# vasabi-root/gaus-slam

Hardware: AMD Instinct MI355X
Metric: fwd+bwd frames/sec @ 640x480, 500k Gaussians (higher is better)
Workload: dtype f32

## Files before the change

gaus_slam_amd/csrc/gs2d_api.hip:

```cpp
#include "gs2d_common.h"
#include "../../include/gs2d_rasterizer.h"

#include <stdio.h>
#include <stdlib.h>
#include <string.h>
#include <chrono>
#include <string>
#include <atomic>
#include <mutex>
#include <thread>
#if defined(__x86_64__) || defined(__i386__)
#include <immintrin.h>
#endif

namespace {

thread_local std::string g_err;

int fail(const char* what, hipError_t e)
{
    char buf[512];
    snprintf(buf, sizeof(buf), "gs2d: %s: %s", what, hipGetErrorString(e));
    g_err = buf;
    return -1;
// ... 6 lines not shown

#define GS2D_CHECK(expr, what)                        \
    do {                                              \
        hipError_t _e = (expr);                       \
        if (_e != hipSuccess) return fail(what, _e);  \
    } while (0)

#define GS2D_STAGE(what)                                                             \
    do {                                                                             \
        hipError_t _e = hipGetLastError();                                           \
        if (_e != hipSuccess) return fail(what, _e);                                 \
        if (debug) { _e = hipStreamSynchronize(s); if (_e != hipSuccess) return fail(what, _e); } \
    } while (0)

uint32_t higher_msb(uint32_t n)
{
    uint32_t msb = sizeof(n) * 4, step = msb;
    while (step > 1) {
        step /= 2;
        if (n >> msb) msb += step; else msb -= step;
    }
    if (n >> msb) msb++;
    return msb;
}

enum { ST_PREPROCESS = 0, ST_SCAN, ST_DUPLICATE, ST_SORT, ST_RANGES, ST_BLEND_FWD, ST_BLEND_BWD, ST_PREPROCESS_BWD, ST_CULL, ST_COUNT };
struct StageTimer {
    bool enabled = false;
    hipEvent_t ev[ST_COUNT][2];
    bool have_ev = false;
    bool recorded[ST_COUNT] = {};
    void begin(int st, hipStream_t s)
    {
        if (!enabled) return;
        if (!have_ev) {
            for (int i = 0; i < ST_COUNT; i++) { (void)hipEventCreate(&ev[i][0]); (void)hipEventCreate(&ev[i][1]); }
            have_ev = true;
        }
        (void)hipEventRecord(ev[st][0], s);
    }
    void end(int st, hipStream_t s)
    {
        if (!enabled) return;
        (void)hipEventRecord(ev[st][1], s);
        recorded[st] = true;
    }
};
StageTimer g_timer;

std::atomic<int> g_deterministic{0};
std::atomic<int> g_reference_binning{0};
static int launch_ahead_default() { const char* e = getenv("GS2D_LAUNCH_AHEAD"); return (e && e[0] == '0') ? 0 : 1; }
std::atomic<int> g_launch_ahead{launch_ahead_default()};

struct PinnedWord {
    uint32_t* p = nullptr;
    ~PinnedWord() { if (p) (void)hipHostFree(p); }
};
thread_local PinnedWord g_pinned;
struct FwdRecord {
    const void* geom = nullptr;
    const void* bin = nullptr;
    size_t bin_bytes = 0;
    int det = 0, R = 0, P = 0;
    bool clean = false;
};
struct FwdTable {
    static constexpr int N = 64;
    std::mutex m;
    FwdRecord e[N];
    int next = 0;
    void drop(const void* geom) { std::lock_guard<std::mutex> l(m); for (auto& r : e) if (r.geom == geom) r = FwdRecord(); }
    void add(const FwdRecord& r) { std::lock_guard<std::mutex> l(m); e[next] = r; next = (next + 1) % N; }
    bool find(const void* geom, bool take_clean, FwdRecord* out)
    {
        std::lock_guard<std::mutex> l(m);
        for (auto& r : e)
            if (r.geom == geom && geom != nullptr) {
                *out = r;
                if (take_clean) r.clean = false;
                return true;
            }
        return false;
    }
};
FwdTable g_fwd;

struct LastCount { int P = -1, W = 0, H = 0; uint32_t R = 0; };
thread_local LastCount g_last[GS2D_MAX_BATCH];

inline void cpu_relax()
{
#if defined(__x86_64__) || defined(__i386__)
    _mm_pause();
#elif defined(__aarch64__)
    asm volatile("yield" ::: "memory");
#else
    std::this_thread::yield();
#endif
}

}

extern "C" {

const char* gs2d_last_error(void) { return g_err.c_str(); }

void gs2d_stage_timing_enable(int on)
{
    g_timer.enabled = on != 0;
    for (int i = 0; i < ST_COUNT; i++) g_timer.recorded[i] = false;
}

int gs2d_stage_timing_read(float ms[9])
{
    for (int i = 0; i < ST_COUNT; i++) {
        ms[i] = -1.f;
        if (!g_timer.recorded[i]) continue;
        if (hipEventSynchronize(g_timer.ev[i][1]) != hipSuccess) return -1;
        float t = 0.f;
        if (hipEventElapsedTime(&t, g_timer.ev[i][0], g_timer.ev[i][1]) != hipSuccess) return -1;
        ms[i] = t;
    }
    return 0;
}

int gs2d_stage_timing_read_abs(float ms[18])
{
    for (int i = 0; i < 2 * ST_COUNT; i++) ms[i] = -1.f;
    if (!g_timer.recorded[ST_PREPROCESS]) return 0;
    for (int i = 0; i < ST_COUNT; i++) {
        if (!g_timer.recorded[i]) continue;
        if (hipEventSynchronize(g_timer.ev[i][1]) != hipSuccess) return -1;
        for (int e = 0; e < 2; e++) {
            float t = 0.f;
            if (hipEventElapsedTime(&t, g_timer.ev[ST_PREPROCESS][0], g_timer.ev[i][e]) != hipSuccess) {
                if (hipEventElapsedTime(&t, g_timer.ev[i][e], g_timer.ev[ST_PREPROCESS][0]) != hipSuccess) return -1;
                t = -t;
            }
            ms[2 * i + e] = t;
        }
    }
    return 0;
}

void gs2d_set_deterministic(int on) { g_deterministic.store(on != 0); }
int gs2d_get_deterministic(void) { return g_deterministic.load(); }
void gs2d_set_reference_binning(int on) { g_reference_binning.store(on != 0); }
void gs2d_set_launch_ahead(int on) { g_launch_ahead.store(on != 0); }
int gs2d_get_launch_ahead(void) { return g_launch_ahead.load(); }
int gs2d_get_reference_binning(void) { return g_reference_binning.load(); }

#ifndef GS2D_SOURCE_HASH
#define GS2D_SOURCE_HASH "unknown"
#endif
const char* gs2d_build_info(void) { return "gs2d-hip gfx950 strict-fp (fp-contract=off) " __DATE__ " src " GS2D_SOURCE_HASH; }

size_t gs2d_geometry_bytes(int P) { return geom_layout(P).total; }
size_t gs2d_image_bytes(int width, int height) { return img_layout(width, height).total; }
size_t gs2d_binning_bytes(int R) { return bin_layout(R, g_deterministic.load() != 0).total; }

void gs2d_geometry_layout(int P, size_t o[5])
{
    const GeomLayout L = geom_layout(P);
    o[0] = L.depths; o[1] = L.tiles_touched; o[2] = L.point_offsets; o[3] = L.rec; o[4] = L.clamped;
}
void gs2d_binning_layout(int R, size_t o[2])
{
    const BinLayout L = bin_layout(R);
    o[0] = L.point_list; o[1] = L.keys;
}
size_t gs2d_binning_contrib_offset(int R) { return bin_layout(R, g_deterministic.load() != 0).contrib; }
void gs2d_image_layout(int width, int height, size_t o[2])
{
    const ImgLayout L = img_layout(width, height);
    o[0] = L.ranges; o[1] = L.pix;
}

}

namespace {

struct FwdShared {
    int P, D, M, width, height, use_sa, debug;
    const float* background;
    const float *means3D, *shs, *colors_precomp, *opacities, *scales, *rotations, *transMat_precomp;
    float scale_modifier;
    hipStream_t s;
};
struct FwdFrame {
    gs2d_alloc_fn geometry_alloc, binning_alloc, image_alloc;
    void *geometry_user, *binning_user, *image_user;
    const float *viewmatrix, *projmatrix, *cam_pos, *pose_Rt, *pose_quat;
    float* out_color; float* out_others; int* radii;
    char* geom = nullptr; char* bin = nullptr; char* img = nullptr;
    size_t bin_bytes = 0;
    GeomLayout GL; CamParams cam;
    volatile uint32_t* pinned = nullptr;
    bool fused_sort = false;
    int sort_cap = 0;
    bool spec = false;
    bool store_pending = false;
    bool ahead = false;
// ... 91 lines not shown
                                f.pose_Rt, f.pose_quat, scan_tmp, s);
    g_timer.end(ST_PREPROCESS, s);
    GS2D_STAGE("preprocess");

    if (!g_pinned.p) GS2D_CHECK(hipHostMalloc((void**)&g_pinned.p, 64, hipHostMallocCoherent), "hipHostMalloc");
    f.pinned = g_pinned.p + slot;
    f.spec = img_layout(c.width, c.height).tiles <= GS2D_BIN_MAX_TILES;
    if (f.spec) return 0;
    const int nblk = (c.P + 255) / 256;
    uint32_t* total_dev = scan_tmp + nblk + 8;
    *f.pinned = 0xFFFFFFFFu;
    g_timer.begin(ST_SCAN, s);
    gs2d::launch_offsets_blocksums(c.P, scan_tmp, total_dev, g_pinned.p + slot, s);
    g_timer.end(ST_SCAN, s);
    {
        const hipError_t le = hipGetLastError();
        if (le != hipSuccess) return fail("scan", le);
    }
    f.store_pending = true;
    return 0;
}

int fwd_phase_b(const FwdShared& c, FwdFrame& f, int slot, bool allow_ahead = true)
{
    const int debug = c.debug;
    hipStream_t s = c.s;
    const int P = c.P, width = c.width, height = c.height;
    const GeomLayout& GL = f.GL;
    const CamParams& cam = f.cam;
    const ImgLayout IL = img_layout(width, height);
    f.img = (char*)f.image_alloc(f.image_user, IL.total);
    if (!f.img) { (void)wait_total(f, s); return fail_msg("image allocation failed"); }
    LastCount& last = g_last[slot];
    const bool same_shape = last.P == P && last.W == width && last.H == height;
    const size_t guess_R = same_shape ? (size_t)last.R + last.R / 8 + 4096 : (size_t)P * 3 + 4096;
    const int C0 = (int)(guess_R > 0x7fffffffull ? 0x7fffffffull : guess_R);
    const bool det = g_deterministic.load() != 0;
    char* geom = f.geom;
    char* img = f.img;
    float* depths = (float*)(geom + GL.depths);
    uint32_t* tiles_touched = (uint32_t*)(geom + GL.tiles_touched);
    uint32_t* point_offsets = (uint32_t*)(geom + GL.point_offsets);
    ushort4* rect = (ushort4*)(geom + GL.rect);
    uint32_t* scan_tmp = (uint32_t*)(geom + GL.scan_tmp);
    int C = C0;
    const size_t pre_bytes = bin_layout(C0, det, C0).total;
    char* bin_pre = (char*)f.binning_alloc(f.binning_user, pre_bytes);
    if (f.spec) {
        if (!bin_pre) return fail_msg("binning allocation failed");
        const BinLayout B0 = bin_layout(C0, det, C0);
        *f.pinned = 0xFFFFFFFFu;
        const bool ahead = allow_ahead && g_launch_ahead.load() != 0 && !debug && !det;
        uint32_t* total_dev = scan_tmp + (P + 255) / 256 + 8;
        g_timer.begin(ST_DUPLICATE, s);
        gs2d::launch_duplicate(P, rect, depths, tiles_touched, scan_tmp, 0, point_offsets, cam.gx, (uint64_t*)(bin_pre + B0.keys_alt),
                               (uint32_t*)(bin_pre + B0.vals_alt), (uint32_t)C0, (uint32_t*)f.pinned, s, ahead ? total_dev : nullptr);
        g_timer.end(ST_DUPLICATE, s);
        {
            const hipError_t le = hipGetLastError();
            if (le != hipSuccess) return fail("duplicate", le);
        }
        f.store_pending = true;
        if (ahead) {
            const gs2d::DevBin db = {bin_pre, total_dev, (uint32_t)C0, 0};
            uint2* ranges = (uint2*)(img + IL.ranges);
            const int tile_bits = (int)higher_msb((uint32_t)(cam.gx * cam.gy));
            g_timer.begin(ST_SORT, s);
            gs2d::launch_bin_by_tile_dev(db, IL.tiles, tile_bits, ranges, s);
            const long long Rg = same_shape ? (long long)last.R : (long long)C0;
            const int cap_class = gs2d::tile_sort_capacity(Rg, IL.tiles);
            f.sort_cap = gs2d::gs2d_fused_sort_cap(cap_class);
            f.fused_sort = f.sort_cap > 0;
            if (!f.fused_sort) gs2d::launch_tile_depth_sort_dev(db, IL.tiles, ranges, cap_class, 0, s);
            g_timer.end(ST_SORT, s);
            GS2D_STAGE("bin by tile (count on the device)");
            f.ahead = true; f.cap = C0; f.det = false;
            f.bin = bin_pre;
            f.bf.ranges = ranges; f.bf.point_list = nullptr; f.bf.rec = (const float4*)(geom + GL.rec);
            f.bf.out_color = f.out_color; f.bf.out_others = f.out_others; f.bf.pix_state = (float*)(img + IL.pix);
            f.bf.hits = nullptr; f.bf.hits4 = nullptr; f.bf.contrib = nullptr; f.bf.zero = (float4*)(geom + GL.grad_rec);
            f.bf.keys = nullptr; f.bf.keys_alt = nullptr; f.bf.vals_alt = nullptr;
            f.bf.dev = db;
            return 0;
        }
    }
    if (!wait_total(f, s)) return fail_msg("num_rendered read-back failed");
    if (debug) GS2D_CHECK(hipStreamSynchronize(s), f.spec ? "duplicate" : "scan");
    const uint32_t num_rendered_u = *f.pinned;
    if (num_rendered_u == 0xFFFFFFFFu) return fail_msg("num_rendered read-back failed");
    if (num_rendered_u > 0x7fffffffu) return fail_msg("num_rendered overflows int32");
    const int R = (int)num_rendered_u;
    f.R = R;

    last.P = P; last.W = width; last.H = height; last.R = num_rendered_u;
    const bool reuse_pre = bin_pre && R <= C0;
    if (!reuse_pre) C = R;
    const BinLayout BL = bin_layout(R, det, C);
    char* bin = reuse_pre ? bin_pre : (char*)f.binning_alloc(f.binning_user, BL.total);
    if (!bin) return fail_msg("binning allocation failed");
    f.bin = bin;
    f.bin_bytes = BL.total;
    uint32_t* point_list = (uint32_t*)(bin + BL.point_list);
    uint64_t* keys = (uint64_t*)(bin + BL.keys);
    uint32_t* vals_alt = (uint32_t*)(bin + BL.vals_alt);
    uint64_t* keys_alt = (uint64_t*)(bin + BL.keys_alt);
    uint32_t* hist = (uint32_t*)(bin + BL.hist);
    uint2* ranges = (uint2*)(img + IL.ranges);

    const int tile_bits = (int)higher_msb((uint32_t)(cam.gx * cam.gy));
    const int end_bit = 32 + tile_bits;
    const bool one_pass = IL.tiles <= GS2D_BIN_MAX_TILES;
    const int passes = one_pass ? 1 : (end_bit - 32 + 7) / 8;
    uint64_t* k_unsorted = (passes & 1) ? keys_alt : keys;
    uint32_t* v_unsorted = (passes & 1) ? vals_alt : point_list;
    if (!f.spec) {
        g_timer.begin(ST_DUPLICATE, s);
        gs2d::launch_duplicate(P, rect, depths, tiles_touched, scan_tmp, 1, point_offsets, cam.gx, k_unsorted, v_unsorted, 0xFFFFFFFFu,
                               nullptr, s);
        g_timer.end(ST_DUPLICATE, s);
    } else if (!reuse_pre) {
        gs2d::launch_duplicate(P, rect, depths, tiles_touched, scan_tmp, 0, point_offsets, cam.gx, k_unsorted, v_unsorted, (uint32_t)C,
// ... 556 lines not shown
```

gaus_slam_amd/csrc/gs2d_binning.hip:

```cpp
#include "gs2d_common.h"
#include "gs2d_scan.h"
#include "gs2d_tile_sort.h"

#include <stdlib.h>

namespace {

__global__ void __launch_bounds__(SCAN_T) scan_reduce_kernel(const uint32_t* __restrict__ in, int n, uint32_t* __restrict__ block_sums)
{
    const int base = blockIdx.x * GS2D_SCAN_ITEMS + threadIdx.x * SCAN_PER_T;
    uint32_t s = 0;
#pragma unroll
    for (int i = 0; i < SCAN_PER_T; i++)
        if (base + i < n) s += in[base + i];
    uint32_t total;
    block_incl_scan(s, &total);
    if (threadIdx.x == 0) block_sums[blockIdx.x] = total;
}

__global__ void __launch_bounds__(SCAN_T) scan_blocksums_kernel(uint32_t* __restrict__ block_sums, int nblocks, uint32_t* __restrict__ total_out,
                                                                uint32_t* __restrict__ total_host)
{
    scan_blocksums_body(block_sums, nblocks, total_out, total_host);
}
// ... 359 lines not shown
bin_scatter_kernel(const uint64_t* __restrict__ keys_in, const uint32_t* __restrict__ vals_in, uint64_t* __restrict__ keys_out,
                   uint32_t* __restrict__ vals_out, int n, int ntiles, int nbits, const uint32_t* __restrict__ offs_excl,
                   const uint32_t* __restrict__ tile_total, int nblocks, uint2* __restrict__ ranges)
{
    bin_scatter_body<ITEMS>(keys_in, vals_in, keys_out, vals_out, n, ntiles, nbits, offs_excl, tile_total, nblocks, ranges);
}
__global__ void __launch_bounds__(BIN_T) bin_scatter_batch_kernel(int ntiles, int nbits, const gs2d::BinFrames tab)
{
    const gs2d::BinFrame& f = tab.f[blockIdx.y];
    if (f.nblocks == 0) return;
    bin_scatter_body<BIN_ITEMS>(f.keys_unsorted, f.vals_unsorted, f.keys, f.point_list, f.R, ntiles, nbits, f.hist,
                                f.hist + (size_t)ntiles * f.nblocks, f.nblocks, f.ranges);
}

struct DevBinPtrs {
    int R, nblocks;
    const uint64_t* keys_unsorted; const uint32_t* vals_unsorted;
    uint64_t* keys; uint32_t* point_list; uint64_t* keys_alt; uint32_t* vals_alt; uint32_t* hist;
};
__device__ __forceinline__ bool dev_bin_ptrs(const gs2d::DevBin& db, DevBinPtrs* o, int items)
{
    const uint32_t R = *db.R_dev;
    if (R > db.cap) return false;
    const BinLayout L = bin_layout((int)R, db.det != 0, (int)db.cap);
    o->R = (int)R;
    o->nblocks = ((int)R + items - 1) / items;
    o->keys = (uint64_t*)(db.base + L.keys); o->point_list = (uint32_t*)(db.base + L.point_list);
    o->keys_alt = (uint64_t*)(db.base + L.keys_alt); o->vals_alt = (uint32_t*)(db.base + L.vals_alt);
    o->keys_unsorted = o->keys_alt; o->vals_unsorted = o->vals_alt;
    o->hist = (uint32_t*)(db.base + L.hist);
    return true;
}
template <int ITEMS>
__global__ void __launch_bounds__(BIN_T) bin_hist_dev_kernel(const gs2d::DevBin db, int ntiles)
{
    DevBinPtrs p;
    if (!dev_bin_ptrs(db, &p, ITEMS)) return;
    bin_hist_body<ITEMS>(p.keys_unsorted, p.R, ntiles, p.hist, p.nblocks);
}
__global__ void __launch_bounds__(256) bin_row_scan_dev_kernel(const gs2d::DevBin db, int ntiles, int items)
{
    DevBinPtrs p;
    if (!dev_bin_ptrs(db, &p, items)) return;
    bin_row_scan_body(p.hist, ntiles, p.nblocks, p.hist + (size_t)ntiles * p.nblocks);
}
template <int ITEMS>
__global__ void __launch_bounds__(BIN_T) bin_scatter_dev_kernel(const gs2d::DevBin db, int ntiles, int nbits, uint2* __restrict__ ranges)
{
    DevBinPtrs p;
    if (!dev_bin_ptrs(db, &p, ITEMS)) return;
    bin_scatter_body<ITEMS>(p.keys_unsorted, p.vals_unsorted, p.keys, p.point_list, p.R, ntiles, nbits, p.hist,
                     p.hist + (size_t)ntiles * p.nblocks, p.nblocks, ranges);
}
__global__ void __launch_bounds__(256)
tile_depth_sort_dev_kernel(const gs2d::DevBin db, const uint2* __restrict__ ranges, int cap, int write_keys)
{
    extern __shared__ uint32_t dyn[];
    __shared__ uint32_t wcnt[4][256];
    DevBinPtrs p;
    if (!dev_bin_ptrs(db, &p, BIN_ITEMS) || p.R == 0) return;
    tile_depth_sort_body(blockIdx.x, dyn, wcnt, ranges, p.keys, p.point_list, p.keys_alt, p.vals_alt, cap, 1, write_keys);
}

__global__ void __launch_bounds__(256)
tile_depth_sort_kernel(const uint2* __restrict__ ranges, uint64_t* __restrict__ keys, uint32_t* __restrict__ vals,
                       uint64_t* __restrict__ keys_alt, uint32_t* __restrict__ vals_alt, int cap, int packed, int write_keys)
{
    extern __shared__ uint32_t dyn[];
    __shared__ uint32_t wcnt[4][256];
    tile_depth_sort_body(blockIdx.x, dyn, wcnt, ranges, keys, vals, keys_alt, vals_alt, cap, packed, write_keys);
}
__global__ void __launch_bounds__(256) tile_depth_sort_batch_kernel(int cap, int write_keys, const gs2d::BinFrames tab)
{
    const gs2d::BinFrame& f = tab.f[blockIdx.y];
    extern __shared__ uint32_t dyn[];
    __shared__ uint32_t wcnt[4][256];
    if (f.R > 0) tile_depth_sort_body(blockIdx.x, dyn, wcnt, f.ranges, f.keys, f.point_list, f.keys_alt, f.vals_alt, cap, 1, write_keys);
}

__global__ void __launch_bounds__(256) tile_ranges_kernel(int L, const uint64_t* __restrict__ keys, uint2* __restrict__ ranges)
{
    const int idx = blockIdx.x * 256 + threadIdx.x;
    if (idx >= L) return;
    const uint32_t cur = (uint32_t)(keys[idx] >> 32);
    if (idx == 0) ranges[cur].x = 0;
    else {
        const uint32_t prev = (uint32_t)(keys[idx - 1] >> 32);
        if (cur != prev) { ranges[prev].y = idx; ranges[cur].x = idx; }
    }
    if (idx == L - 1) ranges[cur].y = L;
}

}

namespace gs2d {

int bin_items_for(long long count, int tiles)
{
    static const int forced = [] { const char* e = getenv("GS2D_BIN_ITEMS_FORCE"); return e ? atoi(e) : 0; }();
    if (forced == 4096 || forced == 8192 || forced == 16384) return forced;
    return tiles > 2560 && count >= 8192LL * 128 ? 8192 : BIN_ITEMS;
}

static size_t bin_lds_bytes(int tiles) { return 4 * (size_t)(tiles + 2 * (tiles + (tiles & 1))); }
static int bin_grid(int nblocks) { return nblocks > 0 ? 8 * ((nblocks + 7) / 8) : 1; }

// ... 24 lines not shown
                      uint32_t capacity, uint32_t* total_host, hipStream_t s, uint32_t* total_dev)
{
    hipLaunchKernelGGL(duplicate_kernel, dim3((P + 255) / 256), dim3(256), 0, s, P, rect, depths, tiles_touched, block_sums, scanned,
                       point_offsets, gx, keys, vals, capacity, total_host, total_dev);
}

void launch_sort_pairs(int R, uint64_t* keys_a, uint32_t* vals_a, uint64_t* keys_b, uint32_t* vals_b, int begin_bit,
                       int end_bit, uint32_t* hist, size_t hist_elems, hipStream_t s)
{
    if (R <= 0) return;
    const int nblocks = (R + GS2D_SORT_ITEMS - 1) / GS2D_SORT_ITEMS;
    uint32_t* scan_tmp = hist + hist_elems;
    const int passes = (end_bit - begin_bit + 7) / 8;
    uint64_t* kin = (passes & 1) ? keys_b : keys_a;
    uint32_t* vin = (passes & 1) ? vals_b : vals_a;
    uint64_t* kout = (passes & 1) ? keys_a : keys_b;
    uint32_t* vout = (passes & 1) ? vals_a : vals_b;
    for (int p = 0; p < passes; p++) {
        const int shift = begin_bit + 8 * p;
        hipLaunchKernelGGL(radix_hist_kernel, dim3(nblocks), dim3(SORT_T), 0, s, kin, R, shift, hist, nblocks);
        launch_inclusive_scan(hist, hist, (int)hist_elems, scan_tmp, nullptr, s);
        hipLaunchKernelGGL(radix_scatter_kernel, dim3(nblocks), dim3(SORT_T), 0, s, kin, vin, kout, vout, R, shift, hist,
                           nblocks);
        uint64_t* tk = kin; kin = kout; kout = tk;
        uint32_t* tv = vin; vin = vout; vout = tv;
    }
}

bool launch_bin_by_tile(int R, int tiles, int nbits, const uint64_t* keys_in, const uint32_t* vals_in, uint64_t* keys_out,
                        uint32_t* vals_out, uint32_t* hist, uint2* ranges, hipStream_t s)
{
    if (tiles > GS2D_BIN_MAX_TILES) return false;
    const int items = bin_items_for(R, tiles);
    const int nblocks = (R + items - 1) / items;
    const size_t hist_elems = (size_t)tiles * nblocks;
    uint32_t* tile_total = hist + hist_elems;
    GS2D_BIN_DISPATCH(items, hipLaunchKernelGGL((bin_hist_kernel<I>), dim3(bin_grid(nblocks)), dim3(BIN_T), (size_t)tiles * 4, s, keys_in, R, tiles, hist, nblocks));
    hipLaunchKernelGGL(bin_row_scan_kernel, dim3((tiles + 3) / 4), dim3(256), 0, s, hist, tiles, nblocks, tile_total);
    GS2D_BIN_DISPATCH(items, hipLaunchKernelGGL((bin_scatter_kernel<I>), dim3(bin_grid(nblocks)), dim3(BIN_T), (size_t)bin_lds_bytes(tiles), s, keys_in, vals_in, keys_out,
                                                vals_out, R, tiles, nbits, hist, tile_total, nblocks, ranges));
    return true;
}

void launch_bin_by_tile_dev(const DevBin& db, int tiles, int nbits, uint2* ranges, hipStream_t s)
{
    const int items = bin_items_for((long long)db.cap, tiles);
    int grid = ((int)db.cap + items - 1) / items;
    if (grid < 1) grid = 1;
    GS2D_BIN_DISPATCH(items, hipLaunchKernelGGL((bin_hist_dev_kernel<I>), dim3(bin_grid(grid)), dim3(BIN_T), (size_t)tiles * 4, s, db, tiles));
    hipLaunchKernelGGL(bin_row_scan_dev_kernel, dim3((tiles + 3) / 4), dim3(256), 0, s, db, tiles, items);
    GS2D_BIN_DISPATCH(items, hipLaunchKernelGGL((bin_scatter_dev_kernel<I>), dim3(bin_grid(grid)), dim3(BIN_T), (size_t)bin_lds_bytes(tiles), s, db, tiles, nbits, ranges));
}

void launch_tile_depth_sort_dev(const DevBin& db, int tiles, const uint2* ranges, int cap_class, int write_keys, hipStream_t s)
{
    if (tiles <= 0) return;
    hipLaunchKernelGGL(tile_depth_sort_dev_kernel, dim3(tiles), dim3(256), (size_t)cap_class * 16, s, db, ranges, cap_class, write_keys);
}

int tile_sort_capacity(long long R, int tiles)
{
    if (tiles <= 0) return 1536;
    const int want = (int)((R * 13) / ((long long)tiles * 10));
    return want <= 1536 ? 1536 : (want <= 2048 ? 2048 : (want <= 3072 ? 3072 : 4096));
}

void launch_tile_depth_sort(int R, int tiles, const uint2* ranges, uint64_t* keys, uint32_t* vals, uint64_t* keys_alt,
                            uint32_t* vals_alt, int packed, int write_keys, hipStream_t s)
{
    if (R <= 0 || tiles <= 0) return;
    const int cap = tile_sort_capacity(R, tiles);
    hipLaunchKernelGGL(tile_depth_sort_kernel, dim3(tiles), dim3(256), (size_t)cap * 16, s, ranges, keys, vals, keys_alt,
                       vals_alt, cap, packed, write_keys);
}

void launch_duplicate_batch(int P, int K, int gx, const BinFrames& tab, hipStream_t s)
{
    hipLaunchKernelGGL(duplicate_batch_kernel, dim3((P + 255) / 256, K), dim3(256), 0, s, P, gx, tab);
}

void launch_bin_sort_batch(int P, int K, int tiles, int gx, int nbits, BinFrames& tab, int write_keys, bool depth_sort, hipStream_t s)
{
    int max_blocks = 0;
    long long max_R = 0;
    for (int k = 0; k < K; k++) {
        tab.f[k].nblocks = (tab.f[k].R + BIN_ITEMS - 1) / BIN_ITEMS;
        max_blocks = tab.f[k].nblocks > max_blocks ? tab.f[k].nblocks : max_blocks;
        max_R = tab.f[k].R > max_R ? tab.f[k].R : max_R;
        if (tab.f[k].R == 0) (void)hipMemsetAsync(tab.f[k].ranges, 0, sizeof(uint2) * (size_t)tiles, s);
    }
    (void)P; (void)gx;
    if (max_blocks == 0) return;
    hipLaunchKernelGGL(bin_hist_batch_kernel, dim3(bin_grid(max_blocks), K), dim3(BIN_T), (size_t)tiles * 4, s, tiles, tab);
    hipLaunchKernelGGL(bin_row_scan_batch_kernel, dim3((tiles + 3) / 4, K), dim3(256), 0, s, tiles, tab);
    hipLaunchKernelGGL(bin_scatter_batch_kernel, dim3(bin_grid(max_blocks), K), dim3(BIN_T), (size_t)bin_lds_bytes(tiles), s, tiles, nbits, tab);
    if (!depth_sort) return;
    const int cap = tile_sort_capacity(max_R, tiles);
    hipLaunchKernelGGL(tile_depth_sort_batch_kernel, dim3(tiles, K), dim3(256), (size_t)cap * 16, s, cap, write_keys, tab);
}

void launch_tile_ranges(int R, const uint64_t* keys, uint2* ranges, int tiles, hipStream_t s)
{
    (void)hipMemsetAsync(ranges, 0, sizeof(uint2) * (size_t)tiles, s);
    if (R > 0) hipLaunchKernelGGL(tile_ranges_kernel, dim3((R + 255) / 256), dim3(256), 0, s, R, keys, ranges);
}

// ... 2 lines not shown
```

gaus_slam_amd/csrc/gs2d_common.h:

```cpp
#pragma once
#include <hip/hip_runtime.h>
#include <stddef.h>
#include <stdint.h>

#define GS2D_TILE 16
#define GS2D_TILE_PIX 256
#define GS2D_NEAR_N 0.2f
#define GS2D_FAR_N 100.0f
#define GS2D_FILTER_INV_SQ 100.0f

#define GS2D_REC_F4 5
#define GS2D_REC_FLOATS 20

#define GS2D_GRAD_FLOATS 20

enum { PS_TFINAL = 0, PS_M1, PS_M2, PS_MEDIAN, PS_STD, PS_LAST, PS_MEDC, PS_PLANES };

__host__ __device__ static inline size_t gs2d_align_up(size_t v, size_t a) { return (v + a - 1) / a * a; }

struct GeomLayout {
    size_t depths, tiles_touched, point_offsets, rec, clamped, scan_tmp, grad_rec, rect, total;
};
struct BinLayout {
    size_t point_list, hits, hits4, keys, vals_alt, keys_alt, hist, det_inv, det_slots, contrib, total;
    size_t hist_elems;
};
struct ImgLayout {
    size_t ranges, pix, total;
    int tiles;
};

#define GS2D_SCAN_ITEMS 1024
#define GS2D_SORT_ITEMS 2048
#ifndef GS2D_BIN_ITEMS
#define GS2D_BIN_ITEMS 4096
#endif
#define GS2D_BIN_MAX_TILES 4096

static inline GeomLayout geom_layout(int P)
{
    GeomLayout L;
    size_t o = 0;
    const size_t p = (size_t)(P > 0 ? P : 1);
    L.depths = o; o = gs2d_align_up(o + 4 * p, 256);
    L.tiles_touched = o; o = gs2d_align_up(o + 4 * p, 256);
    L.point_offsets = o; o = gs2d_align_up(o + 4 * p, 256);
    L.rec = o; o = gs2d_align_up(o + 4 * GS2D_REC_FLOATS * p, 256);
    L.clamped = o; o = gs2d_align_up(o + 3 * p, 256);
    const size_t nblk = (p + 255) / 256;
    L.scan_tmp = o; o = gs2d_align_up(o + 4 * (nblk + 64), 256);
    L.grad_rec = o; o = gs2d_align_up(o + 4 * GS2D_GRAD_FLOATS * p, 256);
    L.rect = o; o = gs2d_align_up(o + 8 * p, 256);
    L.total = o;
    return L;
}

__host__ __device__ static inline BinLayout bin_layout(int R, bool det = false, int C = -1)
{
    BinLayout L;
    const size_t r = (size_t)(R > 0 ? R : 1);
    const size_t c = (C >= 0 && (size_t)C > r) ? (size_t)C : r;
    auto fixed_part = [det](size_t n, BinLayout* out) -> size_t {
        size_t o = 0;
        const size_t point_list = o; o = gs2d_align_up(o + 4 * n, 256);
        const size_t hits = o; o = gs2d_align_up(o + 8 * n, 256);
        const size_t hits4 = o; o = gs2d_align_up(o + 4 * n, 256);
        const size_t keys = o; o = gs2d_align_up(o + 8 * n, 256);
        const size_t nblk = (n + GS2D_SORT_ITEMS - 1) / GS2D_SORT_ITEMS;
        const size_t hist_elems = 256 * nblk;
        const size_t bin_elems = (size_t)GS2D_BIN_MAX_TILES * ((n + GS2D_BIN_ITEMS - 1) / GS2D_BIN_ITEMS);
        const size_t cap_elems = hist_elems > bin_elems ? hist_elems : bin_elems;
        const size_t scan_blk = (cap_elems + GS2D_SCAN_ITEMS - 1) / GS2D_SCAN_ITEMS;
        const size_t hist = o; o = gs2d_align_up(o + 4 * (cap_elems + scan_blk + 64 + GS2D_BIN_MAX_TILES), 256);
        size_t det_inv = o, det_slots = o;
        if (det) {
            o = gs2d_align_up(o + 4 * n, 256);
            det_slots = o; o = gs2d_align_up(o + 4 * (size_t)GS2D_GRAD_FLOATS * 4 * n, 256);
        }
        const size_t contrib = o; o = gs2d_align_up(o + 4 * n, 256);
        if (out) {
            out->point_list = point_list; out->hits = hits; out->hits4 = hits4; out->keys = keys; out->hist = hist;
            out->hist_elems = hist_elems; out->det_inv = det_inv; out->det_slots = det_slots; out->contrib = contrib;
        }
        return o;
    };
    (void)fixed_part(r, &L);
    size_t o = fixed_part(c, nullptr);
    L.vals_alt = o; o = gs2d_align_up(o + 4 * c, 256);
    L.keys_alt = o; o = gs2d_align_up(o + 8 * c, 256);
// ... 34 lines not shown
    if (!(rho_max >= 0.f)) return f;
    f.rl = __builtin_amdgcn_sqrtf(rho_max * (1.0f / GS2D_FILTER_INV_SQ)) + 0.5f;
    f.kind = 2;
    const float a = rho_max * (q2.x * q2.x + q2.y * q2.y), zz = q2.z * q2.z;
    if (!(a <= 0.9f * zz) || !(q2.z > 0.f)) return f;
    const float inv = __builtin_amdgcn_rcpf(a - zz);
    const float f0 = rho_max * inv, f2 = -inv;
    f.cx = f0 * (q0.x * q2.x + q0.y * q2.y) + f2 * (q0.z * q2.z);
    f.cy = f0 * (q1.x * q2.x + q1.y * q2.y) + f2 * (q1.z * q2.z);
    const float ux = q0.y * q2.z - q0.z * q2.y, uy = q0.z * q2.x - q0.x * q2.z, uz = q0.x * q2.y - q0.y * q2.x;
    const float vx = q1.y * q2.z - q1.z * q2.y, vy = q1.z * q2.x - q1.x * q2.z, vz = q1.x * q2.y - q1.y * q2.x;
    const float k = rho_max * (inv * inv);
    const float hx = k * ((ux * ux + uy * uy) - rho_max * (uz * uz));
    const float hy = k * ((vx * vx + vy * vy) - rho_max * (vz * vz));
    if (!(hx == hx) || !(hy == hy)) return f;
    f.ex = __builtin_amdgcn_sqrtf(fmaxf(hx, 0.f)); f.ey = __builtin_amdgcn_sqrtf(fmaxf(hy, 0.f));
    f.mx = 0.1f + 0.002f * f.ex + 1e-4f * fabsf(f.cx); f.my = 0.1f + 0.002f * f.ey + 1e-4f * fabsf(f.cy);
    f.kind = 1;
    return f;
}

namespace gs2d {
void launch_preprocess_fwd(int P, int D, int M, const float* means3D, const float* scales, float scale_modifier,
                           const float* rotations, const float* opacities, const float* shs,
                           const float* transMat_precomp, const float* colors_precomp, const CamParams& cam,
                           int* radii, float* depths, float4* rec, uint32_t* tiles_touched, ushort4* rect, uint8_t* clamped,
                           const float* pose_Rt, const float* pose_q, uint32_t* block_sums, hipStream_t s);
void launch_preprocess_bwd(int first, int P, int D, int M, const float* means3D, const float4* rec, const int* radii,
                           const float* shs, const uint8_t* clamped, const float* scales, const float* rotations,
                           const CamParams& cam, const float* grad_rec, float* dL_dtransMat, float* dL_dnormal,
                           float* dL_dcolor, float* dL_dopacity, float* dL_dsh, float* dL_dmean2D,
                           float* dL_dmean3D, float* dL_dscale, float* dL_drot, const float* pose_Rt, const float* pose_q,
                           float* dL_dpose, int need_record, float* pose_partials, hipStream_t s);
void launch_preprocess_bwd_pose(int P, const float* means3D, const int* radii, const float* scales, const float* rotations,
                                const CamParams& cam, const float* dense_T, const float* dense_m2d, const float* pose_Rt,
                                const float* pose_q, float* dL_dpose, hipStream_t s);
void launch_mark_visible(int P, const float* means3D, const float* vm, uint8_t* present, hipStream_t s);
void launch_pose_quat(const float* pose_Rt, float* q_out, hipStream_t s);
void launch_inclusive_scan(const uint32_t* in, uint32_t* out, int n, uint32_t* tmp, uint32_t* total_out, hipStream_t s,
                           uint32_t* total_host = nullptr);
void launch_offsets_blocksums(int P, uint32_t* block_sums, uint32_t* total_dev, uint32_t* total_host, hipStream_t s);
void launch_duplicate(int P, const ushort4* rect, const float* depths, const uint32_t* tiles_touched,
                      const uint32_t* block_sums, int scanned, uint32_t* point_offsets, int gx, uint64_t* keys, uint32_t* vals,
                      uint32_t capacity, uint32_t* total_host, hipStream_t s, uint32_t* total_dev = nullptr);
void launch_sort_pairs(int R, uint64_t* keys_a, uint32_t* vals_a, uint64_t* keys_b, uint32_t* vals_b, int begin_bit,
                       int end_bit, uint32_t* hist, size_t hist_elems, hipStream_t s);
struct DevBin {
    char* base;
    const uint32_t* R_dev;
    uint32_t cap;
    int det;
};
void launch_bin_by_tile_dev(const DevBin& db, int tiles, int nbits, uint2* ranges, hipStream_t s);
void launch_tile_depth_sort_dev(const DevBin& db, int tiles, const uint2* ranges, int cap_class, int write_keys, hipStream_t s);
bool launch_bin_by_tile(int R, int tiles, int nbits, const uint64_t* keys_in, const uint32_t* vals_in, uint64_t* keys_out,
                        uint32_t* vals_out, uint32_t* hist, uint2* ranges, hipStream_t s);
void launch_tile_depth_sort(int R, int tiles, const uint2* ranges, uint64_t* keys, uint32_t* vals, uint64_t* keys_alt,
                            uint32_t* vals_alt, int packed, int write_keys, hipStream_t s);
void launch_tile_ranges(int R, const uint64_t* keys, uint2* ranges, int tiles, hipStream_t s);
struct PreFwdFrame {
    const float *vm, *pm, *campos;
    int* radii; float* depths; float4* rec; uint32_t* tiles_touched; ushort4* rect; uint8_t* clamped; uint32_t* block_sums;
};
struct PreFwdFrames { PreFwdFrame f[8]; };
struct PreBwdFrame {
    const float *vm, *pm, *campos;
    int W, H;
    const float4* rec; const int* radii; const uint8_t* clamped; const float* grad_rec;
    float *dL_dtransMat, *dL_dnormal, *dL_dcolor, *dL_dopacity, *dL_dsh, *dL_dmean2D, *dL_dmean3D, *dL_dscale, *dL_drot;
};
struct PreBwdFrames { PreBwdFrame f[8]; };
void launch_preprocess_fwd_batch(int P, int K, int D, int M, const float* means3D, const float* scales, float scale_modifier,
                                 const float* rotations, const float* opacities, const float* shs, const float* transMat_precomp,
                                 const float* colors_precomp, const CamParams& cam0, const PreFwdFrames& tab, hipStream_t s);
void launch_preprocess_bwd_batch(int P, int K, int D, int M, const float* means3D, const float* shs, const float* scales,
                                 const float* rotations, int need_record, const PreBwdFrames& tab, hipStream_t s);
void launch_sum_frames(int P, int K, int M, const PreBwdFrames& tab, hipStream_t s);

struct BinFrame {
    const ushort4* rect; const float* depths; const uint32_t* tiles_touched;
    const uint32_t* block_sums;
    uint32_t* total_host;
    uint32_t capacity;
    uint32_t* point_offsets;
    uint64_t* keys_unsorted; uint32_t* vals_unsorted;
    uint64_t* keys; uint32_t* point_list;
    uint64_t* keys_alt; uint32_t* vals_alt;
    uint32_t* hist;
    uint2* ranges;
    int R, nblocks;
};
struct BinFrames { BinFrame f[8]; };
void launch_duplicate_batch(int P, int K, int gx, const BinFrames& tab, hipStream_t s);
void launch_bin_sort_batch(int P, int K, int tiles, int gx, int nbits, BinFrames& tab, int write_keys, bool depth_sort, hipStream_t s);
int tile_sort_capacity(long long R, int tiles);
#define GS2D_FUSED_SORT_CAP 1536
#define GS2D_FUSED_SORT_CAP_IDX 3072
static inline int gs2d_fused_sort_cap(int cap_class)
{
    return cap_class <= GS2D_FUSED_SORT_CAP ? GS2D_FUSED_SORT_CAP : (cap_class <= GS2D_FUSED_SORT_CAP_IDX ? GS2D_FUSED_SORT_CAP_IDX : 0);
}
static inline size_t gs2d_fused_sort_lds(int sort_cap) { return (size_t)sort_cap * (sort_cap > GS2D_FUSED_SORT_CAP ? 8 : 16) + 4096; }

#define GS2D_MAX_BATCH 8
struct BlendFwdFrame {
    const uint2* ranges; uint32_t* point_list; const float4* rec;
// ... 25 lines not shown
```

gaus_slam_amd/rasterizer.py:

```python
import contextlib
import ctypes as C
from typing import NamedTuple

import torch
import torch.nn as nn

from . import _lib
from ._host import Chunk as _Chunk, chunks as _chunks, on_device as _on_device, ptr as _ptr, stream_ptr as _stream_ptr

NUM_CHANNELS = 3
_BWD_BLEND, _BWD_PREPROCESS = _lib.BWD_BLEND, _lib.BWD_PREPROCESS
_BWD_POSE_ONLY = _lib.BWD_BLEND | _lib.BWD_PREPROCESS | _lib.BWD_POSE_4X4


def _check_cuda(t, name):
    if not t.is_cuda:
        raise RuntimeError(f"{name} must be a CUDA tensor")


def _f32c(t):
    if t is None:
        return None
    return t.contiguous() if t.dtype == torch.float32 else t.float().contiguous()

# ... 166 lines not shown
    M = sh.size(1) if sh.size(0) != 0 else 0
    has_transmat = transMat_precomp.numel() != 0
    outs = [_grad_outputs(P, M, dev, lean, has_transmat, grad_sink if k == 0 else None) for k in range(K)]
    if P != 0:
        keep = [_f32c(t) for t in (background, means3D, sh, colors, scales, rotations, transMat_precomp)]
        bg_, m3_, sh_, col_, sc_, rot_, tm_ = keep
        dc_ = [_f32c(dL_dout_color[k]) for k in range(K)]
        do_ = [_f32c(dL_dout_others[k]) for k in range(K)]
        vm_ = _f32c(viewmatrices).reshape(K, 16)
        pm_ = _f32c(projmatrices).reshape(K, 16)
        cp_ = _f32c(camposs).reshape(K, 3)
        radii_ = radii.contiguous()
        fr = (_lib.FrameGrad * K)()
        for k in range(K):
            f = fr[k]
            f.viewmatrix, f.projmatrix, f.campos = vm_[k].data_ptr(), pm_[k].data_ptr(), cp_[k].data_ptr()
            f.tan_fovx, f.tan_fovy = float(tan_fovxs[k]), float(tan_fovys[k])
            f.radii = radii_[k].data_ptr()
            f.geom_buffer, f.binning_buffer, f.img_buffer = _ptr(geomBuffers[k]), _ptr(binningBuffers[k]), _ptr(imageBuffers[k])
            f.num_rendered = int(Rs[k])
            f.dL_dpix, f.dL_depths = dc_[k].data_ptr(), do_[k].data_ptr()
            (f.dL_dmean2D, f.dL_dnormal, f.dL_dopacity, f.dL_dcolor, f.dL_dmean3D, f.dL_dtransMat, f.dL_dsh, f.dL_dscale,
             f.dL_drot) = map(_ptr, outs[k])
        _lib.call("gs2d_backward_batch", dev, K, fr, int(bool(accumulate)), P, int(degree), M, _ptr(bg_), W, H, _ptr(m3_),
                  _ptr(sh_), _ptr(col_), _ptr(sc_), float(scale_modifier), _ptr(rot_), _ptr(tm_), int(bool(use_sa)),
                  int(bool(debug)))
    return [_returned_grads(o) for o in outs]


def set_deterministic(on=True):
    _lib.lib().gs2d_set_deterministic(int(bool(on)))


def is_deterministic():
    return bool(_lib.lib().gs2d_get_deterministic())


def set_reference_binning(on=True):
    _lib.lib().gs2d_set_reference_binning(int(bool(on)))


def is_reference_binning():
    return bool(_lib.lib().gs2d_get_reference_binning())


def set_launch_ahead(on=True):
    _lib.lib().gs2d_set_launch_ahead(int(bool(on)))


def is_launch_ahead():
    return bool(_lib.lib().gs2d_get_launch_ahead())


def mark_visible(means3D, viewmatrix, projmatrix):
    P = means3D.size(0)
    present = torch.zeros((P,), dtype=torch.bool, device=means3D.device)
    if P != 0:
        m3_, vm_, pm_ = _f32c(means3D), _f32c(viewmatrix), _f32c(projmatrix)
        _lib.call("gs2d_mark_visible", means3D.device, P, m3_.data_ptr(), vm_.data_ptr(), pm_.data_ptr(), present.data_ptr())
    return present


class _Sink:
    views = None
    chunk_rows = None
    on_chunk = None
    armed = False
    consumed = False


_SINK = _Sink()


@contextlib.contextmanager
def grad_sink(views, chunk_rows=None, on_chunk=None):
    if _SINK.armed:
        raise RuntimeError("grad_sink contexts cannot be nested")
    _SINK.views, _SINK.armed, _SINK.consumed = views, True, False
    _SINK.chunk_rows, _SINK.on_chunk = chunk_rows, on_chunk
    try:
        yield
    finally:
        _SINK.views, _SINK.armed, _SINK.consumed = None, False, False
        _SINK.chunk_rows, _SINK.on_chunk = None, None


def _take_sink():
    if not _SINK.armed:
        return None, None, None
    if _SINK.consumed:
        raise RuntimeError("a second rasterizer backward ran inside one grad_sink context: only one operator call per "
                           "direct-gradient backward is supported (render once per keyframe, or use direct_grads=False)")
    _SINK.consumed = True
    return _SINK.views, _SINK.chunk_rows, _SINK.on_chunk


def _cpu_copy(args):
    return tuple(a.detach().cpu().clone() if isinstance(a, torch.Tensor) else a for a in args)


def _with_snapshot(fn, args, kwargs, path, message):
    cpu_args = _cpu_copy(args)
    try:
        return fn(*args, **kwargs)
    except Exception as ex:
        torch.save(cpu_args, path)
# ... 201 lines not shown
```

Baseline: 2371.

## Bin Gaussians by tile directly from screen rects, skipping key duplication

```diff
diff --git a/gaus_slam_amd/csrc/gs2d_api.hip b/gaus_slam_amd/csrc/gs2d_api.hip
--- a/gaus_slam_amd/csrc/gs2d_api.hip
+++ b/gaus_slam_amd/csrc/gs2d_api.hip
@@ -82,6 +82,8 @@
 std::atomic<int> g_reference_binning{0};
 static int launch_ahead_default() { const char* e = getenv("GS2D_LAUNCH_AHEAD"); return (e && e[0] == '0') ? 0 : 1; }
 std::atomic<int> g_launch_ahead{launch_ahead_default()};
+static int rect_binning_default() { const char* e = getenv("GS2D_RECT_BINNING"); return (e && e[0] == '0') ? 0 : 1; }
+std::atomic<int> g_rect_binning{rect_binning_default()};
 
 struct PinnedWord {
     uint32_t* p = nullptr;
@@ -177,8 +179,12 @@
 void gs2d_set_deterministic(int on) { g_deterministic.store(on != 0); }
 int gs2d_get_deterministic(void) { return g_deterministic.load(); }
 void gs2d_set_reference_binning(int on) { g_reference_binning.store(on != 0); }
-void gs2d_set_launch_ahead(int on) { g_launch_ahead.store(on != 0); }
-int gs2d_get_launch_ahead(void) { return g_launch_ahead.load(); }
+void gs2d_set_launch_ahead(int on)
+{
+    g_launch_ahead.store(on != 0);
+    g_rect_binning.store(on == 2 ? 0 : rect_binning_default());
+}
+int gs2d_get_launch_ahead(void) { return g_launch_ahead.load() == 0 ? 0 : (g_rect_binning.load() != 0 ? 1 : 2); }
 int gs2d_get_reference_binning(void) { return g_reference_binning.load(); }
 
 #ifndef GS2D_SOURCE_HASH
@@ -376,9 +382,15 @@
         *f.pinned = 0xFFFFFFFFu;
         const bool ahead = allow_ahead && g_launch_ahead.load() != 0 && !debug && !det;
         uint32_t* total_dev = scan_tmp + (P + 255) / 256 + 8;
+        uint32_t* const rect_table = (uint32_t*)(bin_pre + B0.vals_alt);
+        const bool rect_bin = ahead && g_rect_binning.load() != 0 && gs2d::rect_bin_waves(IL.tiles) != 0 && gs2d::rect_bin_table_bytes(P, IL.tiles) <= B0.total - B0.vals_alt;
         g_timer.begin(ST_DUPLICATE, s);
-        gs2d::launch_duplicate(P, rect, depths, tiles_touched, scan_tmp, 0, point_offsets, cam.gx, (uint64_t*)(bin_pre + B0.keys_alt),
-                               (uint32_t*)(bin_pre + B0.vals_alt), (uint32_t)C0, (uint32_t*)f.pinned, s, ahead ? total_dev : nullptr);
+        if (rect_bin)
+            gs2d::launch_bin_count_rect(P, rect, tiles_touched, scan_tmp, point_offsets, cam.gx, IL.tiles, rect_table,
+                                        (uint32_t*)f.pinned, total_dev, s);
+        else
+            gs2d::launch_duplicate(P, rect, depths, tiles_touched, scan_tmp, 0, point_offsets, cam.gx, (uint64_t*)(bin_pre + B0.keys_alt),
+                                   (uint32_t*)(bin_pre + B0.vals_alt), (uint32_t)C0, (uint32_t*)f.pinned, s, ahead ? total_dev : nullptr);
         g_timer.end(ST_DUPLICATE, s);
         {
             const hipError_t le = hipGetLastError();
@@ -390,7 +402,8 @@
             uint2* ranges = (uint2*)(img + IL.ranges);
             const int tile_bits = (int)higher_msb((uint32_t)(cam.gx * cam.gy));
             g_timer.begin(ST_SORT, s);
-            gs2d::launch_bin_by_tile_dev(db, IL.tiles, tile_bits, ranges, s);
+            if (rect_bin) gs2d::launch_bin_scatter_rect(db, P, rect, depths, tiles_touched, cam.gx, IL.tiles, rect_table, ranges, s);
+            else gs2d::launch_bin_by_tile_dev(db, IL.tiles, tile_bits, ranges, s);
             const long long Rg = same_shape ? (long long)last.R : (long long)C0;
             const int cap_class = gs2d::tile_sort_capacity(Rg, IL.tiles);
             f.sort_cap = gs2d::gs2d_fused_sort_cap(cap_class);
diff --git a/gaus_slam_amd/csrc/gs2d_binning.hip b/gaus_slam_amd/csrc/gs2d_binning.hip
--- a/gaus_slam_amd/csrc/gs2d_binning.hip
+++ b/gaus_slam_amd/csrc/gs2d_binning.hip
@@ -435,6 +435,226 @@
     bin_scatter_body<ITEMS>(p.keys_unsorted, p.vals_unsorted, p.keys, p.point_list, p.R, ntiles, nbits, p.hist,
                      p.hist + (size_t)ntiles * p.nblocks, p.nblocks, ranges);
 }
+constexpr int RECT_ITEMS = GS2D_RECT_ITEMS;
+constexpr uint32_t RECT_BIG = 48;
+constexpr int RECT_SUB = 4;
+
+template <int NW>
+__device__ __forceinline__ uint32_t rect_block_incl_scan(uint32_t v, uint32_t* total)
+{
+    __shared__ uint32_t wsum[NW];
+    const int lane = threadIdx.x & 63, wave = threadIdx.x >> 6;
+    const uint32_t inc = wave_incl_scan(v, lane);
+    __syncthreads();
+    if (lane == 63) wsum[wave] = inc;
+    __syncthreads();
+    uint32_t base = 0, all = 0;
+#pragma unroll
+    for (int w = 0; w < NW; w++) {
+        const uint32_t x = wsum[w];
+        if (w < wave) base += x;
+        all += x;
+    }
+    if (total) *total = all;
+    return inc + base;
+}
+
+__device__ __forceinline__ uint32_t rect_tile(const ushort4 r, uint32_t k, uint32_t gx)
+{
+    const uint32_t w = (uint32_t)r.z - (uint32_t)r.x;
+    const uint32_t yy = k / w;
+    return ((uint32_t)r.y + yy) * gx + (uint32_t)r.x + (k - yy * w);
+}
+
+template <typename Add>
+__device__ __forceinline__ void wave_count_rects(const ushort4 r, uint32_t n, uint32_t gx, int lane, Add add)
+{
+    if (n - 1u < RECT_BIG)
+        for (uint32_t y = r.y; y < r.w; y++)
+            for (uint32_t x = r.x; x < r.z; x++) add(y * gx + x);
+    uint64_t big = __ballot(n > RECT_BIG);
+    while (big) {
+        const int j = __builtin_ctzll(big);
+        big &= big - 1;
+        const uint32_t nj = (uint32_t)__builtin_amdgcn_readlane((int)n, j);
+        const uint32_t lo = (uint32_t)__builtin_amdgcn_readlane((int)((uint32_t)r.x | ((uint32_t)r.y << 16)), j);
+        const uint32_t hi = (uint32_t)__builtin_amdgcn_readlane((int)((uint32_t)r.z | ((uint32_t)r.w << 16)), j);
+        const ushort4 rj = make_ushort4((unsigned short)(lo & 0xffffu), (unsigned short)(lo >> 16), (unsigned short)(hi & 0xffffu),
+                                        (unsigned short)(hi >> 16));
+        for (uint32_t k = (uint32_t)lane; k < nj; k += 64) add(rect_tile(rj, k, gx));
+    }
+}
+
+template <int NW>
+__global__ void __launch_bounds__(64 * NW)
+bin_count_rect_kernel(int P, const ushort4* __restrict__ rect, const uint32_t* __restrict__ tiles_touched,
+                      const uint32_t* __restrict__ block_sums, uint32_t* __restrict__ point_offsets, int gx, int ntiles,
+                      uint32_t* __restrict__ hist, int nblocks, uint32_t* __restrict__ total_host, uint32_t* __restrict__ total_dev)
+{
+    extern __shared__ uint32_t lds[];
+    constexpr int T = 64 * NW;
+    const int blk = bin_block_of(blockIdx.x, nblocks);
+    if (blk < 0) return;
+    const int lane = threadIdx.x & 63;
+    for (int t = threadIdx.x; t < ntiles; t += T) lds[t] = 0;
+    constexpr int PER_T = RECT_ITEMS / T;
+    const int first = blk * RECT_ITEMS + (int)threadIdx.x * PER_T;
+    uint32_t n[PER_T];
+    ushort4 r[PER_T];
+    uint32_t mysum = 0;
+#pragma unroll
+    for (int i = 0; i < PER_T; i++) {
+        const int g = first + i;
+        n[i] = g < P ? tiles_touched[g] : 0u;
+        r[i] = rect[min(g, P - 1)];
+        mysum += n[i];
+    }
+    uint32_t before = 0;
+    for (int b = threadIdx.x; b < blk * (RECT_ITEMS / 256); b += T) before += block_sums[b];
+    uint32_t block_offset, own_total;
+    (void)rect_block_incl_scan<NW>(before, &block_offset);
+    uint32_t run = block_offset + rect_block_incl_scan<NW>(mysum, &own_total) - mysum;
+    if (total_host != nullptr && blk == nblocks - 1 && threadIdx.x == 0) {
+        const uint32_t total = block_offset + own_total;
+        if (total_dev != nullptr) *total_dev = total;
+        __hip_atomic_store(total_host, total == 0xFFFFFFFFu ? 0xFFFFFFFEu : total, __ATOMIC_RELAXED, __HIP_MEMORY_SCOPE_SYSTEM);
+    }
+#pragma unroll
+    for (int i = 0; i < PER_T; i++) {
+        run += n[i];
+        if (first + i < P) point_offsets[first + i] = run;
+    }
+#pragma unroll
+    for (int i = 0; i < PER_T; i++)
+        wave_count_rects(r[i], n[i], (uint32_t)gx, lane, [&](uint32_t t) { atomicAdd(&lds[t], 1u); });
+    __syncthreads();
+    for (int t = threadIdx.x; t < ntiles; t += T) hist[(size_t)t * nblocks + blk] = lds[t];
+}
+
+template <int NW>
+__global__ void __launch_bounds__(64 * NW)
+bin_scatter_rect_kernel(const gs2d::DevBin db, int P, const ushort4* __restrict__ rect, const float* __restrict__ depths,
+                        const uint32_t* __restrict__ tiles_touched, int gx, int ntiles, const uint32_t* __restrict__ offs_excl,
+                        const uint32_t* __restrict__ tile_total, int nblocks, uint2* __restrict__ ranges)
+{
+    extern __shared__ uint32_t lds[];
+    constexpr int T = 64 * NW;
+    constexpr int CHUNKS = RECT_ITEMS / T;
+    const uint32_t R = *db.R_dev;
+    if (R > db.cap) return;
+    const int blk = bin_block_of(blockIdx.x, nblocks);
+    if (blk < 0) return;
+    uint2* const out = reinterpret_cast<uint2*>(db.base + bin_layout((int)R, db.det != 0, (int)db.cap).keys);
+    const int lane = threadIdx.x & 63, wave = threadIdx.x >> 6;
+    const int nt2 = ntiles + (ntiles & 1);
+    uint32_t* const cnt_words = lds + ntiles;
+    for (int t = threadIdx.x; t < (NW / 2) * nt2; t += T) cnt_words[t] = 0;
+    uint32_t* const mine = cnt_words + wave * (nt2 >> 1);
+    const int g0 = blk * RECT_ITEMS + wave * (CHUNKS * 64);
+    uint32_t n[CHUNKS], dbits[CHUNKS], incl[CHUNKS];
+    ushort4 r[CHUNKS];
+#pragma unroll
+    for (int c = 0; c < CHUNKS; c++) {
+        const int g = g0 + c * 64 + lane;
+        const int ci = min(g, P - 1);
+        n[c] = g < P ? tiles_touched[ci] : 0u;
+        r[c] = rect[ci];
+        dbits[c] = __float_as_uint(depths[ci]);
+    }
+#pragma unroll
+    for (int c = 0; c < CHUNKS; c++) incl[c] = n[c];
+#pragma unroll
+    for (int d = 1; d < 64; d <<= 1)
+#pragma unroll
+        for (int c = 0; c < CHUNKS; c++) {
+            const uint32_t up = __shfl_up(incl[c], d, 64);
+            if (lane >= d) incl[c] += up;
+        }
+    __syncthreads();
+#pragma unroll
+    for (int c = 0; c < CHUNKS; c++)
+        wave_count_rects(r[c], n[c], (uint32_t)gx, lane, [&](uint32_t d) { atomicAdd(&mine[d >> 1], 1u << (16 * (d & 1u))); });
+    __syncthreads();
+    {
+        const int K = (ntiles + T - 1) / T;
+        const int t0 = min(ntiles, (int)threadIdx.x * K), t1 = min(ntiles, t0 + K);
+        uint32_t mysum = 0;
+        for (int t = t0; t < t1; t++) mysum += tile_total[t];
+        uint32_t running = rect_block_incl_scan<NW>(mysum, nullptr) - mysum;
+        uint16_t* const c16 = reinterpret_cast<uint16_t*>(cnt_words);
+        for (int t = t0; t < t1; t++) {
+            const uint32_t tot = tile_total[t];
+            lds[t] = running + offs_excl[(size_t)t * nblocks + blk];
+            uint32_t acc = 0;
+#pragma unroll
+            for (int w = 0; w < NW; w++) {
+                const uint32_t cw = c16[w * nt2 + t];
+                c16[w * nt2 + t] = (uint16_t)acc;
+                acc += cw;
+            }
+            if (blk == 0) ranges[t] = tot ? make_uint2(running, running + tot) : make_uint2(0u, 0u);
+            running += tot;
+        }
+    }
+    __syncthreads();
+    const uint64_t lt_mask = lane == 0 ? 0ull : (~0ull >> (64 - lane));
+#pragma unroll
+    for (int c = 0; c < CHUNKS; c++) {
+        const uint32_t total = (uint32_t)__builtin_amdgcn_readlane((int)incl[c], 63);
+        const uint32_t rlo = (uint32_t)r[c].x | ((uint32_t)r[c].y << 16), rhi = (uint32_t)r[c].z | ((uint32_t)r[c].w << 16);
+        const uint32_t excl = incl[c] - n[c];
+#pragma unroll 1
+        for (uint32_t s = 0; s < total; s += 64 * RECT_SUB) {
+            uint32_t d[RECT_SUB], dep[RECT_SUB], id[RECT_SUB], rk[RECT_SUB], nw[RECT_SUB], dstb[RECT_SUB];
+            bool valid[RECT_SUB];
+#pragma unroll
+            for (int q = 0; q < RECT_SUB; q++) {
+                const uint32_t p = s + 64 * q + (uint32_t)lane;
+                valid[q] = p < total;
+                int j = 0;
+#pragma unroll
+                for (int st = 32; st >= 1; st >>= 1) {
+                    const uint32_t v = (uint32_t)__shfl((int)incl[c], j + st - 1, 64);
+                    if (v <= p) j += st;
+                }
+                const uint32_t excl_j = (uint32_t)__shfl((int)excl, j, 64);
+                const uint32_t lo = (uint32_t)__shfl((int)rlo, j, 64), hi = (uint32_t)__shfl((int)rhi, j, 64);
+                dep[q] = (uint32_t)__shfl((int)dbits[c], j, 64);
+                const ushort4 rj = make_ushort4((unsigned short)(lo & 0xffffu), (unsigned short)(lo >> 16),
+                                                (unsigned short)(hi & 0xffffu), (unsigned short)(hi >> 16));
+                d[q] = valid[q] ? rect_tile(rj, p - excl_j, (uint32_t)gx) : 0u;
+                id[q] = (uint32_t)(g0 + c * 64 + j);
+            }
+#pragma unroll
+            for (int q = 0; q < RECT_SUB; q++) {
+                rk[q] = 0; nw[q] = 1; dstb[q] = 0;
+                if (valid[q]) {
+                    rk[q] = __hip_atomic_fetch_add(&mine[d[q] >> 1], 1u << (16 * (d[q] & 1u)), __ATOMIC_RELAXED, __HIP_MEMORY_SCOPE_WORKGROUP);
+                    nw[q] = __hip_atomic_load(&mine[d[q] >> 1], __ATOMIC_RELAXED, __HIP_MEMORY_SCOPE_WORKGROUP);
+                    dstb[q] = lds[d[q]];
+                }
+            }
+#pragma unroll
+            for (int q = 0; q < RECT_SUB; q++) {
+                if (s + 64 * q >= total) break;
+                const uint32_t sh = 16 * (d[q] & 1u);
+                uint32_t rank = (rk[q] >> sh) & 0xffffu;
+                const uint32_t now = (nw[q] >> sh) & 0xffffu;
+                uint64_t clash = __ballot(valid[q] && now != rank + 1u);
+                while (clash) {
+                    const int leader = __builtin_ctzll(clash);
+                    const uint32_t dl = (uint32_t)__builtin_amdgcn_readlane((int)d[q], leader);
+                    const uint32_t nowl = (uint32_t)__builtin_amdgcn_readlane((int)now, leader);
+                    const uint64_t m = __ballot(valid[q] && d[q] == dl);
+                    if (valid[q] && d[q] == dl) rank = nowl - (uint32_t)__popcll(m) + (uint32_t)__popcll(m & lt_mask);
+                    clash &= ~m;
+                }
+                if (valid[q]) out[dstb[q] + rank] = make_uint2(dep[q], id[q]);
+            }
+        }
+    }
+}
+
 __global__ void __launch_bounds__(256)
 tile_depth_sort_dev_kernel(const gs2d::DevBin db, const uint2* __restrict__ ranges, int cap, int write_keys)
 {
@@ -565,6 +785,35 @@
     GS2D_BIN_DISPATCH(items, hipLaunchKernelGGL((bin_scatter_dev_kernel<I>), dim3(bin_grid(grid)), dim3(BIN_T), (size_t)bin_lds_bytes(tiles), s, db, tiles, nbits, ranges));
 }
 
+int rect_bin_blocks(int P) { return (P + RECT_ITEMS - 1) / RECT_ITEMS; }
+size_t rect_bin_table_bytes(int P, int tiles) { return 4 * ((size_t)tiles * rect_bin_blocks(P) + (size_t)tiles); }
+
+static size_t rect_lds_bytes(int tiles, int nw) { return 4 * (size_t)tiles + 2 * (size_t)nw * (size_t)(tiles + (tiles & 1)); }
+int rect_bin_waves(int tiles) { return rect_lds_bytes(tiles, 16) <= 65536 ? 16 : (rect_lds_bytes(tiles, 8) <= 65536 ? 8 : 0); }
+
+void launch_bin_count_rect(int P, const ushort4* rect, const uint32_t* tiles_touched, const uint32_t* block_sums,
+                           uint32_t* point_offsets, int gx, int tiles, uint32_t* table, uint32_t* total_host, uint32_t* total_dev,
+                           hipStream_t s)
+{
+    const int nblocks = rect_bin_blocks(P);
+    hipLaunchKernelGGL((bin_count_rect_kernel<16>), dim3(bin_grid(nblocks)), dim3(1024), (size_t)tiles * 4, s, P, rect, tiles_touched,
+                       block_sums, point_offsets, gx, tiles, table, nblocks, total_host, total_dev);
+}
+
+void launch_bin_scatter_rect(const DevBin& db, int P, const ushort4* rect, const float* depths, const uint32_t* tiles_touched,
+                             int gx, int tiles, uint32_t* table, uint2* ranges, hipStream_t s)
+{
+    const int nblocks = rect_bin_blocks(P);
+    uint32_t* tile_total = table + (size_t)tiles * nblocks;
+    hipLaunchKernelGGL(bin_row_scan_kernel, dim3((tiles + 3) / 4), dim3(256), 0, s, table, tiles, nblocks, tile_total);
+    if (rect_bin_waves(tiles) == 16)
+        hipLaunchKernelGGL((bin_scatter_rect_kernel<16>), dim3(bin_grid(nblocks)), dim3(1024), rect_lds_bytes(tiles, 16), s, db, P, rect,
+                           depths, tiles_touched, gx, tiles, table, tile_total, nblocks, ranges);
+    else
+        hipLaunchKernelGGL((bin_scatter_rect_kernel<8>), dim3(bin_grid(nblocks)), dim3(512), rect_lds_bytes(tiles, 8), s, db, P, rect,
+                           depths, tiles_touched, gx, tiles, table, tile_total, nblocks, ranges);
+}
+
 void launch_tile_depth_sort_dev(const DevBin& db, int tiles, const uint2* ranges, int cap_class, int write_keys, hipStream_t s)
 {
     if (tiles <= 0) return;
diff --git a/gaus_slam_amd/csrc/gs2d_common.h b/gaus_slam_amd/csrc/gs2d_common.h
--- a/gaus_slam_amd/csrc/gs2d_common.h
+++ b/gaus_slam_amd/csrc/gs2d_common.h
@@ -35,6 +35,7 @@
 #ifndef GS2D_BIN_ITEMS
 #define GS2D_BIN_ITEMS 4096
 #endif
+#define GS2D_RECT_ITEMS 2048
 #define GS2D_BIN_MAX_TILES 4096
 
 static inline GeomLayout geom_layout(int P)
@@ -175,6 +176,14 @@
     int det;
 };
 void launch_bin_by_tile_dev(const DevBin& db, int tiles, int nbits, uint2* ranges, hipStream_t s);
+int rect_bin_blocks(int P);
+int rect_bin_waves(int tiles);
+size_t rect_bin_table_bytes(int P, int tiles);
+void launch_bin_count_rect(int P, const ushort4* rect, const uint32_t* tiles_touched, const uint32_t* block_sums,
+                           uint32_t* point_offsets, int gx, int tiles, uint32_t* table, uint32_t* total_host, uint32_t* total_dev,
+                           hipStream_t s);
+void launch_bin_scatter_rect(const DevBin& db, int P, const ushort4* rect, const float* depths, const uint32_t* tiles_touched,
+                             int gx, int tiles, uint32_t* table, uint2* ranges, hipStream_t s);
 void launch_tile_depth_sort_dev(const DevBin& db, int tiles, const uint2* ranges, int cap_class, int write_keys, hipStream_t s);
 bool launch_bin_by_tile(int R, int tiles, int nbits, const uint64_t* keys_in, const uint32_t* vals_in, uint64_t* keys_out,
                         uint32_t* vals_out, uint32_t* hist, uint2* ranges, hipStream_t s);
diff --git a/gaus_slam_amd/rasterizer.py b/gaus_slam_amd/rasterizer.py
--- a/gaus_slam_amd/rasterizer.py
+++ b/gaus_slam_amd/rasterizer.py
@@ -242,6 +242,14 @@
     return bool(_lib.lib().gs2d_get_launch_ahead())
 
 
+def set_rect_binning(on=True):
+    _lib.lib().gs2d_set_launch_ahead(1 if on else 2)
+
+
+def is_rect_binning():
+    return _lib.lib().gs2d_get_launch_ahead() == 1
+
+
 def mark_visible(means3D, viewmatrix, projmatrix):
     P = means3D.size(0)
     present = torch.zeros((P,), dtype=torch.bool, device=means3D.device)
```

Result: no change. 2417 (median of 3 runs) (+2.0%).
